# musyoku/chainer-speech-recognition

Measured on AMD Instinct MI355X. Metric: utterances/sec (T=1000, 40x3 feat, |V|~3000) CTC train step, higher is better.
Workload: dtype bf16

## Files before the change

chainer-speech-recognition_amd/asr/_lib.py:

```python
import ctypes
import os

import torch

_HERE = os.path.dirname(os.path.abspath(__file__))
_ACT = os.environ.get("ASR_ACT", "").lower()
LIB_PATH = os.environ.get("ASR_HIP_LIB") or os.path.join(os.path.dirname(_HERE),
                                                        "libasr_hip_f16.so" if _ACT in ("f16", "fp16", "float16", "half") else "libasr_hip.so")

_lib = None


def act_dtype():
    return torch.float16 if lib().asr_act_dtype() else torch.bfloat16


def debug_flag(key, default):
    for item in os.environ.get("ASR_DEBUG", "").split(","):
        k, _, v = item.strip().partition("=")
        if k == key and v:
            return int(v)
    return default

c_void_p, c_int, c_float, c_size_t = ctypes.c_void_p, ctypes.c_int, ctypes.c_float, ctypes.c_size_t
# ... 107 lines not shown
    "asr_gru_fwd_state": (c_int, [c_void_p] * 9 + [c_int] * 4 + [c_void_p]),
    "asr_gru_bwd_state": (c_int, [c_void_p] * 13 + [c_int] * 4 + [c_void_p, c_void_p]),
    "asr_sru_ws_bytes": (c_size_t, [c_int] * 3),
    "asr_sru_fwd": (c_int, [c_void_p] * 9 + [c_int] * 4 + [c_void_p, c_size_t]),
    "asr_sru_bwd": (c_int, [c_void_p] * 13 + [c_int] * 4 + [c_void_p, c_size_t]),
    "asr_sru_combine": (c_int, [c_void_p] * 5 + [c_longlong, c_int]),
    "asr_fill_f32": (c_int, [c_void_p, c_void_p, c_longlong, c_float]),
    "asr_sqnorm_acc": (c_int, [c_void_p, c_void_p, c_longlong, c_void_p]),
    "asr_clip_decay_sgd": (c_int, [c_void_p] * 4 + [c_longlong, c_int] + [c_float] * 5 + [c_void_p]),
    "asr_clip_decay_adam": (c_int, [c_void_p] * 5 + [c_longlong] + [c_float] * 7 + [c_void_p, c_int]),
    "asr_sqnorm_partials_count": (c_int, [c_longlong]),
    "asr_gather_abort": (c_int, [c_void_p, c_void_p, c_int, c_void_p, c_void_p]),
    "asr_step_control": (c_int, [c_void_p, c_void_p, c_longlong] + [c_void_p] * 3 + [c_float] * 5 + [c_void_p] * 2 + [c_int]),
    "asr_step_control_scaled": (c_int, [c_void_p, c_void_p, c_longlong] + [c_void_p] * 3 + [c_float] * 5 + [c_void_p] * 2 + [c_int, c_void_p]),
    "asr_adam_ctl": (c_int, [c_void_p] * 5 + [c_longlong] + [c_float] * 4 + [c_void_p]),
    "asr_crelu_fwd": (c_int, [c_void_p] * 3 + [c_longlong, c_int]),
    "asr_crelu_bwd": (c_int, [c_void_p] * 4 + [c_longlong, c_int]),
    "asr_softmax_fwd": (c_int, [c_void_p] * 3 + [c_longlong, c_int, c_int]),
    "asr_softmax_bwd": (c_int, [c_void_p] * 4 + [c_longlong, c_int, c_int]),
    "asr_avgpool_h_fwd": (c_int, [c_void_p] * 3 + [c_longlong, c_int, c_int, c_int]),
    "asr_avgpool_h_bwd": (c_int, [c_void_p] * 3 + [c_longlong, c_int, c_int, c_int]),
    "asr_unpool_h_fwd": (c_int, [c_void_p] * 3 + [c_longlong, c_int, c_int, c_int, c_int]),
    "asr_unpool_h_bwd": (c_int, [c_void_p] * 3 + [c_longlong, c_int, c_int, c_int, c_int]),
    "asr_gaussian_noise": (c_int, [c_void_p] * 3 + [c_longlong, c_float, ctypes.c_uint]),
    "asr_maxpool_h_indexes": (c_int, [c_void_p, c_void_p, c_void_p, c_longlong, c_int, c_int, c_int]),
    "asr_upsample_h_fwd": (c_int, [c_void_p] * 4 + [c_longlong] + [c_int] * 4),
    "asr_upsample_h_bwd": (c_int, [c_void_p] * 4 + [c_longlong] + [c_int] * 4),
    "asr_spp_bins": (c_int, [c_int]),
    "asr_spp_fwd": (c_int, [c_void_p] * 4 + [c_int] * 5),
    "asr_spp_bwd": (c_int, [c_void_p] * 4 + [c_int] * 5),
# ... 43 lines not shown
```

chainer-speech-recognition_amd/asr/_ops.py:

```python
import os

import torch

from . import _lib
from ._lib import check, ptr, stream

BF16 = _lib.act_dtype()
F32 = torch.float32


def _is_bf16(t):
    if t.dtype == BF16:
        return 1
    if t.dtype == F32:
        return 0
    raise TypeError("expected float32 or bfloat16, got %s" % t.dtype)


def gemm_nt(a, b, bias=None, out_dtype=BF16, out=None):
    assert a.dtype == BF16 and b.dtype == BF16 and a.dim() == 2 and b.dim() == 2
    assert a.stride(1) == 1 and b.stride(1) == 1 and a.shape[1] == b.shape[1]
    M, K = a.shape
    N = b.shape[0]
    if out is None:
# ... 503 lines not shown

def clip_decay_adam(p, g, m, v, alpha, beta1, beta2, eps, weight_decay, clip, grad_scale, sqnorm, step):
    rc = _lib.lib().asr_clip_decay_adam(stream(), ptr(p), ptr(g), ptr(m), ptr(v), p.numel(), alpha, beta1, beta2, eps,
                                        weight_decay, clip, grad_scale, ptr(sqnorm), int(step))
    check(rc, "asr_clip_decay_adam")


def abort_words():
    return [buf[1023:1024] for buf in _SYNC.values()]


_ABORT = {}


def gather_abort(dev, poison=None):
    words = [w for w in abort_words() if w.device == dev]
    ptrs = tuple(w.data_ptr() for w in words)
    st = _ABORT.get(dev.index)
    if st is None or st[0] != ptrs:
        table = torch.tensor(list(ptrs) or [0], dtype=torch.int64).to(dev)
        st = _ABORT[dev.index] = [ptrs, table, torch.zeros(1, dtype=torch.int32, device=dev) if st is None else st[2]]
    check(_lib.lib().asr_gather_abort(stream(), ptr(st[1]), len(words), ptr(st[2]), ptr(poison)), "asr_gather_abort")
    return st[2]


def clear_abort_words(dev):
    for w in abort_words():
        if w.device == dev:
            w.zero_()


def step_control(g, partials, clip, grad_scale, alpha, beta1, beta2, applied, ctl, any_abort=None, reserved_index=-1, loss_scale=None):
    if any_abort is None:
        any_abort = gather_abort(g.device)
    rc = _lib.lib().asr_step_control_scaled(stream(), ptr(g), g.numel(), ptr(partials), ptr(any_abort), None, float(clip),
                                            float(grad_scale), float(alpha), float(beta1), float(beta2), ptr(applied), ptr(ctl),
                                            int(reserved_index), None if loss_scale is None else ptr(loss_scale))
    check(rc, "asr_step_control_scaled")


def sqnorm_partials_count(n):
    return int(_lib.lib().asr_sqnorm_partials_count(int(n)))


def adam_ctl(p, g, m, v, beta1, beta2, eps, weight_decay, ctl):
    rc = _lib.lib().asr_adam_ctl(stream(), ptr(p), ptr(g), ptr(m), ptr(v), p.numel(), beta1, beta2, eps, weight_decay, ptr(ctl))
    check(rc, "asr_adam_ctl")


def sgd_ctl(p, g, v, kind, lr, momentum, weight_decay, ctl):
    rc = _lib.lib().asr_sgd_ctl(stream(), ptr(p), ptr(g), ptr(v), p.numel(), int(kind), lr, momentum, weight_decay, ptr(ctl))
    check(rc, "asr_sgd_ctl")


SRU_CHUNKED = [True]


def _sru_ws(T, B, D, dev):
    n = int(_lib.lib().asr_sru_ws_bytes(T, B, D)) if SRU_CHUNKED[0] else 0
    return (torch.empty(n, dtype=torch.uint8, device=dev), n) if n else (None, 0)


# ... 408 lines not shown
```

chainer-speech-recognition_amd/asr/functions.py:

```python
import math
import os

import torch

from . import _ops
from ._lib import debug_flag as _lib_debug
from .link import grad_buffer, grads_queued

BF16, F32 = _ops.BF16, torch.float32


_SIDE = {"streams": {}, "origins": {}, "enabled": True, "dirty": set(), "keep": [], "keep_bytes": 0,
         "join_before_recurrence": _lib_debug("side_join", 0) != 0}
_KEEP_LIMIT = 512
_KEEP_BYTES_LIMIT = int(_lib_debug("side_keep_gb", 48)) << 30


def side_stream():
    if not _SIDE["enabled"]:
        return None
    cur = torch.cuda.current_stream()
    key = cur.cuda_stream
    st = _SIDE["streams"].get(key)
    if st is None:
# ... 359 lines not shown


def conv_weight_matrix_bwd(W):
    return _ops.conv_weight_pack_bwd(W.contiguous())


def conv_weight_matrix_pad8(W):
    Co, Ci, KH, KW = W.shape
    Wp = torch.zeros((Co, 8, KH, KW), dtype=W.dtype, device=W.device)
    Wp[:, :Ci] = W
    return _ops.conv_weight_pack(Wp, Kp=(KH * KW * 8 + 31) // 32 * 32)


def convolution_2d(x, W, b, link, pad=(0, 0), causal=False, out_f32=False):
    pad_h, pad_t = (pad, pad) if isinstance(pad, int) else pad
    w16 = link.compute_copy("w16", W, conv_weight_matrix)
    w16t = link.compute_copy("w16t", W, conv_weight_matrix_t)
    wbwd = link.compute_copy("wbwd", W, conv_weight_matrix_bwd) if _ops.conv_implicit_ok(W.shape[0], W.shape[2], W.shape[3]) else None
    if x.dtype not in (F32, BF16):
        raise TypeError("convolution input must be float32 or bfloat16")
    w16p = link.compute_copy("w16p", W, conv_weight_matrix_pad8) if W.shape[1] < 8 else None
    y = _Conv2D.apply(x, W, b, w16, w16t, wbwd, w16p, int(pad_h), int(pad_t), bool(causal), bool(out_f32))
    return logical4(y)


def convolution_2d_given_weight(x, W, b, link, pad=(0, 0), causal=False, out_f32=False):
    pad_h, pad_t = (pad, pad) if isinstance(pad, int) else pad
    with torch.no_grad():
        w16 = conv_weight_matrix(W.detach())
        w16t = conv_weight_matrix_t(W.detach())
        wbwd = conv_weight_matrix_bwd(W.detach()) if _ops.conv_implicit_ok(W.shape[0], W.shape[2], W.shape[3]) else None
        w16p = conv_weight_matrix_pad8(W.detach()) if W.shape[1] < 8 else None
    y = _Conv2D.apply(x, W, b, w16, w16t, wbwd, w16p, int(pad_h), int(pad_t), bool(causal), bool(out_f32))
    return logical4(y)


# ... 51 lines not shown
        return False
    Co, Ci, KH, KW = wshape
    if not _ops.conv_mp_ok(Ci, KH, KW, Co, k) or Ci >= 8:
        return False
    return x.shape[2] + 2 * pad_h - KH + 1 >= 1 and (x.shape[3] if causal else x.shape[3] + 2 * pad_t - KW + 1) >= 1


def convolution_maxout_pool(x, W, b, link, pad, causal, k, given_weight=False):
    pad_h, pad_t = (pad, pad) if isinstance(pad, int) else pad
    if not convolution_maxout_pool_ok(x, tuple(W.shape), pad, causal, k):
        return None
    if given_weight:
        with torch.no_grad():
            w16q = conv_weight_matrix_pad8_128(W.detach())
    else:
        w16q = link.compute_copy("w16q", W, conv_weight_matrix_pad8_128)
    return logical4(_ConvMaxoutPool.apply(x, W, b, w16q, int(pad_h), int(pad_t), bool(causal), int(k)))


class _Dense(torch.autograd.Function):

    @staticmethod
    def forward(ctx, x2, W, b, w16, w16t, out_f32):
        y = _ops.gemm_nt(x2, w16, b.detach() if b is not None else None, F32 if out_f32 else BF16)
        ctx.save_for_backward(x2, w16t)
        ctx.params = (W, b)
        ctx.need_dx = ctx.needs_input_grad[0]
        if out_f32:
            ctx._asr_mailbox = _GradMailbox(y, b)
        return y

# ... 686 lines not shown
```

chainer-speech-recognition_amd/asr/link.py:

```python
import contextlib
import math

import torch

from . import _lib

F32 = torch.float32
BF16 = _lib.act_dtype()

_WEIGHT_EPOCH = [0]


def bump_weight_epoch():
    _WEIGHT_EPOCH[0] += 1


class Parameter(torch.nn.Parameter):

    def __new__(cls, data=None):
        if data is None:
            data = torch.empty(0, dtype=F32)
        return super().__new__(cls, data, requires_grad=True)


class Link(torch.nn.Module):
    def __init__(self):
        super().__init__()
        object.__setattr__(self, "_compute_cache", {})
        object.__setattr__(self, "_cast_registry", {})

    @contextlib.contextmanager
    def init_scope(self):
        yield

    @property
    def xp(self):
        return torch

    def params(self):
        return self.parameters()

    def namedparams(self):
        for name, p in self.named_parameters():
            yield "/" + name.replace(".", "/"), p
# ... 17 lines not shown
            src = state_dict.get(prefix + name)
            if p is not None and p.numel() == 0 and src is not None and src.numel() > 0:
                p.data = torch.empty(src.shape, dtype=p.dtype, device=p.device)
        super()._load_from_state_dict(state_dict, prefix, *args, **kwargs)
        bump_weight_epoch()

    def compute_copy(self, key, param, maker, layout=None):
        stamp = (_WEIGHT_EPOCH[0], param._version, param.data_ptr())
        hit = self._compute_cache.get(key)
        if hit is not None and hit[0] == stamp:
            _await_copy(hit)
            return hit[1]
        with torch.no_grad():
            value = maker(param.detach())
        self._compute_cache[key] = _made_copy(stamp, value)
        if layout is not None and value.is_cuda:
            self._cast_registry[key] = (param, value, _cast_jobs(param, layout))
        return value


def _made_copy(stamp, value):
    if not value.is_cuda:
        return (stamp, value, None, None)
    cur = torch.cuda.current_stream()
    return (stamp, value, {"stream": cur, "event": None}, {cur.cuda_stream})


def _await_copy(entry):
    if entry[2] is None:
        return
    cur = torch.cuda.current_stream()
# ... 9 lines not shown

def _cast_jobs(param, layout):
    n, shape = param.numel(), tuple(param.shape)
    if layout == "plain":
        return ((0, 0, n // shape[-1], shape[-1], 0),)
    if layout == "t_first":
        return ((0, 0, shape[0], n // shape[0], 1),)
    if layout == "t_last":
        return ((0, 0, n // shape[-1], shape[-1], 1),)
    if layout == "t_each":
        each = shape[-2] * shape[-1]
        return tuple((i * each, i * each, shape[-2], shape[-1], 1) for i in range(n // each))
    raise ValueError(layout)


def refresh_compute_copies(model):
    from . import _lib
    todo, sig = [], []
    for m in model.modules():
        reg = getattr(m, "_cast_registry", None)
        if not reg:
            continue
        for key, (param, out, jobs) in reg.items():
            hit = m._compute_cache.get(key)
            if hit is None or hit[1] is not out or hit[0][2] != param.data_ptr() or not param.is_cuda:
                continue
            todo.append((m, key, param, out))
            sig.append((param.data_ptr(), out.data_ptr(), jobs))
    if not todo:
        return 0
    cached = getattr(model, "_cast_table", None)
    if cached is None or cached[0] != sig:
        rows, tile = [], 0
        for src, dst, jobs in sig:
            for so, do, r, c, t in jobs:
                rows.append([src + 4 * so, dst + 2 * do, r, c, t, tile])
                tile += ((r + 63) // 64) * ((c + 63) // 64)
        table = torch.tensor(rows, dtype=torch.int64).to(todo[0][2].device)
        cached = (sig, table, len(rows), tile)
        object.__setattr__(model, "_cast_table", cached)
    _lib.check(_lib.lib().asr_cast_bf16_many(_lib.stream(), _lib.ptr(cached[1]), cached[2], cached[3]), "asr_cast_bf16_many")
    for m, key, param, out in todo:
        m._compute_cache[key] = _made_copy((_WEIGHT_EPOCH[0], param._version, param.data_ptr()), out)
    return cached[2]


class Chain(Link):
    pass


_GRAD_LISTENER = [None]


def grads_queued(*params):
    if _GRAD_LISTENER[0] is not None:
        _GRAD_LISTENER[0]([p for p in params if p is not None])


def grad_buffer(param):
# ... 89 lines not shown
```

chainer-speech-recognition_amd/asr/optimizers.py:

```python
import torch

from . import _ops
from .link import bump_weight_epoch, refresh_compute_copies

F32 = torch.float32
RESERVED = 64


class GradientClipping(object):
    name = "GradientClipping"

    def __init__(self, threshold):
        self.threshold = threshold


class WeightDecay(object):
    name = "WeightDecay"

    def __init__(self, rate):
        self.rate = rate


class Optimizer(object):
    def __init__(self):
# ... 51 lines not shown
                ls = self._loss_scale_buffer(loss.device)
                if ls is None:
                    loss.backward()
                else:
                    loss.backward(gradient=ls[0].reshape(loss.shape).to(loss.dtype))
            except BaseException:
                if self.communicator is not None:
                    self.communicator.abort_backward()
                from .functions import release_side_keeps
                release_side_keeps(to_allocator=True)
                raise
        self._ensure_flat()
        from .functions import join_side_stream
        join_side_stream()
        P, G = self._flat["P"], self._flat["G"]
        any_abort = _ops.gather_abort(G.device, G[0:1] if self.communicator is not None else None)
        scale = 1.0
        if self.communicator is not None:
            self.communicator.finish_backward(self)
            scale = 1.0 / self.communicator.size
        self.t += 1
        clip, decay = 0.0, 0.0
        for h in self._hooks:
            if isinstance(h, GradientClipping):
                clip = float(h.threshold)
            elif isinstance(h, WeightDecay):
                decay = float(h.rate)
        alpha, beta1, beta2 = self._control_constants()
        _ops.step_control(G, self._flat["partials"], clip, scale, alpha, beta1, beta2, self._flat["applied"], self._flat["ctl"],
                          any_abort, 0, self._loss_scale_buffer(G.device))
        self._step(P, G, decay, self._flat["ctl"])
        bump_weight_epoch()
        refresh_compute_copies(self.target)
        try:
            self._raise_if_previous_step_gave_up()
        finally:
            self._watch_gave_up()

    def _watch_gave_up(self):
        st = self._gave_up
        if st[0] is None:
            st[0] = torch.zeros(1, dtype=F32).pin_memory()
        if st[1] is None or st[1].query():
            st[0].copy_(self._flat["ctl"][6:7], non_blocking=True)
            st[1] = torch.cuda.Event()
            st[1].record()
            st[2] = self.t

# ... 91 lines not shown

    def _carried(self, total, dev, old, previous):
        state = torch.empty(total, dtype=F32, device=dev)
        _ops.fill_(state, 0.0)
        if old is not None and previous is not None and previous.device == dev:
            where = {pid: (o, n) for pid, o, n in zip(old["ids"], old["offsets"], old["numels"])}
            for pid, o, n in zip(self._flat["ids"], self._flat["offsets"], self._flat["numels"]):
                src = where.get(pid)
                if src is not None and src[1] == n:
                    state[o:o + n].copy_(previous[src[0]:src[0] + n])
        return state

    def _step(self, P, G, decay, ctl):
        raise NotImplementedError


class Adam(Optimizer):
    def __init__(self, alpha=0.001, beta1=0.9, beta2=0.999, eps=1e-8):
        super().__init__()
        self.alpha, self.beta1, self.beta2, self.eps = alpha, beta1, beta2, eps

        self.m = self.v = None

    def _init_state(self, total, dev, old):
        self.m = self._carried(total, dev, old, self.m)
        self.v = self._carried(total, dev, old, self.v)

    def _control_constants(self):
        return self.alpha, self.beta1, self.beta2

    def _state_buffers(self):
        return [self.m, self.v]

    def _step(self, P, G, decay, ctl):
        _ops.adam_ctl(P, G, self.m, self.v, self.beta1, self.beta2, self.eps, decay, ctl)


class SGD(Optimizer):
    kind = 0

    def __init__(self, lr=0.01):
        super().__init__()
        self.lr = lr
        self.momentum = 0.0
        self.vel = None

    def _init_state(self, total, dev, old):
        if self.kind:
            self.vel = self._carried(total, dev, old, self.vel)

    def _state_buffers(self):
        return [self.vel]

    def _step(self, P, G, decay, ctl):
        _ops.sgd_ctl(P, G, self.vel, self.kind, self.lr, self.momentum, decay, ctl)


class MomentumSGD(SGD):
    kind = 1

    def __init__(self, lr=0.01, momentum=0.9):
        super().__init__(lr)
        self.momentum = momentum


class NesterovAG(SGD):
    kind = 2

    def __init__(self, lr=0.01, momentum=0.9):
        super().__init__(lr)
# ... 55 lines not shown
```

chainer-speech-recognition_amd/csrc/optim.hip:

```cpp
#include "common.hpp"
#include "../../include/asr_hip.h"

namespace asr {
namespace optim {

__global__ __launch_bounds__(256) void sqnorm_kernel(const float* __restrict__ g, long long n, float* __restrict__ out) {
    __shared__ float scratch[32];
    float s = 0.f;
    for (long long i = blockIdx.x * (long long)blockDim.x + threadIdx.x; i < n; i += (long long)gridDim.x * blockDim.x) {
        const float v = g[i];
        s += v * v;
    }
    s = block_sum(s, scratch);
    if (threadIdx.x == 0) atomicAdd(out, s);
}

__global__ __launch_bounds__(256) void adam_kernel(float* __restrict__ p, const float* __restrict__ g,
                                                   float* __restrict__ m, float* __restrict__ v, long long n, float lr_t,
                                                   float beta1, float beta2, float eps, float decay, float clip,
                                                   float grad_scale, const float* __restrict__ sqnorm) {
    float rate = grad_scale;
    if (sqnorm) {
        if (!isfinite(sqnorm[0])) return;
        if (clip > 0.f) {
// ... 50 lines not shown
    if (threadIdx.x == 0) partials[blockIdx.x] = s;
}

__global__ void gather_abort_kernel(const long long* __restrict__ word_ptrs, int n, int* __restrict__ any_word, float* __restrict__ poison) {
    int any = 0;
    for (int i = 0; i < n; ++i) {
        const int* w = reinterpret_cast<const int*>(word_ptrs[i]);
        if (w && w[0] != 0) any = 1;
    }
    if (any_word) any_word[0] = any;
    if (any && poison) poison[0] = __int_as_float(0x7fc00000);
}

__global__ __launch_bounds__(256) void step_control_kernel(const float* __restrict__ partials, int npartials,
                                                           const int* __restrict__ abort0, const int* __restrict__ abort1,
                                                           float clip, float grad_scale, float alpha, float beta1, float beta2,
                                                           int* __restrict__ applied, float* __restrict__ ctl,
                                                           const float* __restrict__ reserved, float* __restrict__ ls) {
    __shared__ float scratch[32];
    float s = 0.f;
    for (int i = threadIdx.x; i < npartials; i += blockDim.x) s += partials[i];
    const float sq = block_sum(s, scratch);
    if (threadIdx.x != 0) return;
    ctl[4] = sq;
    const float* sqnorm = &sq;
    bool drop = !isfinite(sqnorm[0]);
    bool gave_up = false;
    if (abort0 && abort0[0] != 0) gave_up = true;
    if (abort1 && abort1[0] != 0) gave_up = true;
    if (reserved && !isfinite(reserved[0])) gave_up = true;
    if (gave_up) drop = true;
    if (ls) {
        grad_scale /= ls[0];
        if (drop && !gave_up) {
            if (ls[2] > 0.f) ls[0] = fmaxf(ls[0] * 0.5f, 1.f / 16777216.f);
            ls[1] = 0.f;
            ls[3] += 1.f;
        } else if (!drop) {
            ls[1] += 1.f;
            if (ls[2] > 0.f && ls[1] >= ls[2]) {
                ls[0] = fminf(ls[0] * 2.f, 16777216.f);
                ls[1] = 0.f;
// ... 6 lines not shown
        const float r = clip / norm;
        if (r < 1.f) rate *= r;
    }
    int t = applied[0];
    if (!drop) applied[0] = ++t;
    const double tt = t < 1 ? 1.0 : (double)t;
    const double fix1 = 1.0 - pow((double)beta1, tt), fix2 = 1.0 - pow((double)beta2, tt);
    ctl[0] = drop ? 1.f : 0.f;
    ctl[1] = rate;
    ctl[2] = (float)((double)alpha * sqrt(fix2) / fix1);
    ctl[3] = (float)t;
    ctl[5] = gave_up ? 1.f : 0.f;
    if (gave_up) ctl[6] += 1.f;
}

__global__ __launch_bounds__(256) void adam_ctl_kernel(float* __restrict__ p, const float* __restrict__ g, float* __restrict__ m,
                                                       float* __restrict__ v, long long n, float beta1, float beta2, float eps,
                                                       float decay, const float* __restrict__ ctl) {
    if (ctl[0] != 0.f) return;
    const float rate = ctl[1], lr_t = ctl[2];
    for (long long i = blockIdx.x * (long long)blockDim.x + threadIdx.x; i < n; i += (long long)gridDim.x * blockDim.x) {
        const float pi = p[i];
        const float gi = g[i] * rate + decay * pi;
        float mi = m[i], vi = v[i];
        mi += (1.f - beta1) * (gi - mi);
        vi += (1.f - beta2) * (gi * gi - vi);
        m[i] = mi;
        v[i] = vi;
        p[i] = pi - lr_t * mi / (sqrtf(vi) + eps);
    }
}

__global__ __launch_bounds__(256) void sgd_ctl_kernel(float* __restrict__ p, const float* __restrict__ g, float* __restrict__ v,
                                                      long long n, int kind, float lr, float mu, float decay,
                                                      const float* __restrict__ ctl) {
    if (ctl[0] != 0.f) return;
    const float rate = ctl[1];
    for (long long i = blockIdx.x * (long long)blockDim.x + threadIdx.x; i < n; i += (long long)gridDim.x * blockDim.x) {
        const float pi = p[i];
        const float gi = g[i] * rate + decay * pi;
        if (kind == 0) {
            p[i] = pi - lr * gi;
        } else {
            const float vi = mu * v[i] - lr * gi;
            v[i] = vi;
            p[i] = kind == 1 ? pi + vi : pi + mu * mu * vi - (1.f + mu) * lr * gi;
        }
    }
}

__global__ void fill_kernel(float* __restrict__ p, long long n, float value) {
    for (long long i = blockIdx.x * (long long)blockDim.x + threadIdx.x; i < n; i += (long long)gridDim.x * blockDim.x) p[i] = value;
}

}
}

using namespace asr;
using namespace asr::optim;

static inline int grid_for(long long n) {
// ... 35 lines not shown
    hipLaunchKernelGGL(sgd_kernel, dim3(grid_for(n)), dim3(256), 0, (hipStream_t)stream, p, g, v, n, kind, lr, momentum,
                       weight_decay, clip_threshold, grad_scale, sqnorm);
    ASR_LAUNCH_CHECK();
    return ASR_OK;
}

extern "C" int asr_sqnorm_partials_count(long long n) { return grid_for(n); }

extern "C" int asr_gather_abort(void* stream, const long long* word_ptrs, int n, int* any_word, float* poison) {
    if (n < 0 || (n > 0 && !word_ptrs) || (!any_word && !poison)) return ASR_ERR_BAD_ARG;
    hipLaunchKernelGGL(gather_abort_kernel, dim3(1), dim3(1), 0, (hipStream_t)stream, word_ptrs, n, any_word, poison);
    ASR_LAUNCH_CHECK();
    return ASR_OK;
}

extern "C" int asr_step_control_scaled(void* stream, const float* g, long long n, float* partials, const int* abort0, const int* abort1,
                                       float clip_threshold, float grad_scale, float alpha, float beta1, float beta2,
                                       int* applied_steps, float* ctl, int reserved_index, float* loss_scale) {
    if (!g || n <= 0 || !partials || !applied_steps || !ctl || reserved_index >= n) return ASR_ERR_BAD_ARG;
    const int blocks = grid_for(n);
    hipLaunchKernelGGL(sqnorm_partials_kernel, dim3(blocks), dim3(256), 0, (hipStream_t)stream, g, n, partials);
    hipLaunchKernelGGL(step_control_kernel, dim3(1), dim3(256), 0, (hipStream_t)stream, (const float*)partials, blocks, abort0,
                       abort1, clip_threshold, grad_scale, alpha, beta1, beta2, applied_steps, ctl,
                       reserved_index >= 0 ? g + reserved_index : (const float*)nullptr, loss_scale);
    ASR_LAUNCH_CHECK();
    return ASR_OK;
}

extern "C" int asr_step_control(void* stream, const float* g, long long n, float* partials, const int* abort0, const int* abort1,
                                float clip_threshold, float grad_scale, float alpha, float beta1, float beta2,
                                int* applied_steps, float* ctl, int reserved_index) {
    return asr_step_control_scaled(stream, g, n, partials, abort0, abort1, clip_threshold, grad_scale, alpha, beta1, beta2,
                                   applied_steps, ctl, reserved_index, nullptr);
}

extern "C" int asr_adam_ctl(void* stream, float* p, const float* g, float* m, float* v, long long n, float beta1, float beta2,
                            float eps, float weight_decay, const float* ctl) {
    if (!p || !g || !m || !v || !ctl || n <= 0) return ASR_ERR_BAD_ARG;
    hipLaunchKernelGGL(adam_ctl_kernel, dim3(grid_for(n)), dim3(256), 0, (hipStream_t)stream, p, g, m, v, n, beta1, beta2, eps,
                       weight_decay, ctl);
    ASR_LAUNCH_CHECK();
    return ASR_OK;
}

extern "C" int asr_sgd_ctl(void* stream, float* p, const float* g, float* v, long long n, int kind, float lr, float momentum,
                           float weight_decay, const float* ctl) {
    if (!p || !g || !ctl || n <= 0 || kind < 0 || kind > 2 || (kind > 0 && !v)) return ASR_ERR_BAD_ARG;
    hipLaunchKernelGGL(sgd_ctl_kernel, dim3(grid_for(n)), dim3(256), 0, (hipStream_t)stream, p, g, v, n, kind, lr, momentum,
                       weight_decay, ctl);
    ASR_LAUNCH_CHECK();
    return ASR_OK;
}
```

include/asr_hip.h:

```cpp
#ifndef ASR_HIP_H
#define ASR_HIP_H
#include <stddef.h>
#include <stdint.h>
#ifdef __cplusplus
extern "C" {
#endif

int asr_version(void);
int asr_act_dtype(void);
int asr_stream_delay(void* stream, int microseconds);
int asr_occupy_cus(void* stream, int microseconds, int lds_bytes, int blocks);
int asr_stream_traffic(void* stream, int microseconds, int lds_bytes, int blocks, void* buf, long long bytes);

size_t asr_ctc_workspace_bytes(int T, int B, int V, int Lmax, int gram);
int asr_ctc_forward(void* stream, const float* xs, const int32_t* label_unigram, const int32_t* label_bigram,
                    const int32_t* x_len, const int32_t* l_len, int T, int B, int V, int Lmax, int blank,
                    float* loss_per_utt, float* loss_mean, void* workspace, size_t workspace_bytes);
int asr_ctc_forward_lse(void* stream, const float* xs, const int32_t* label_unigram, const int32_t* label_bigram,
                        const int32_t* x_len, const int32_t* l_len, int T, int B, int V, int Lmax, int blank, float* loss_per_utt,
                        float* loss_mean, void* workspace, size_t workspace_bytes, const float* row_lse);
int asr_ctc_backward(void* stream, const float* xs, const int32_t* x_len, int T, int B, int V, int Lmax, int gram,
                     const float* gy, int gy_per_utt, float scale, float* grad, const void* workspace,
                     size_t workspace_bytes);
int asr_ctc_loss_grad(void* stream, const float* xs, const int32_t* label_unigram, const int32_t* label_bigram,
// ... 178 lines not shown
                        float grad_scale, const float* sqnorm, int step);
int asr_clip_decay_sgd(void* stream, float* p, const float* g, float* v, long long n, int kind, float lr, float momentum,
                       float weight_decay, float clip_threshold, float grad_scale, const float* sqnorm);
int asr_sqnorm_partials_count(long long n);
int asr_gather_abort(void* stream, const long long* word_ptrs, int n, int* any_word, float* poison);
int asr_step_control(void* stream, const float* g, long long n, float* partials, const int* abort0, const int* abort1,
                     float clip_threshold, float grad_scale, float alpha, float beta1, float beta2, int* applied_steps,
                     float* ctl, int reserved_index);
int asr_step_control_scaled(void* stream, const float* g, long long n, float* partials, const int* abort0, const int* abort1,
                            float clip_threshold, float grad_scale, float alpha, float beta1, float beta2, int* applied_steps,
                            float* ctl, int reserved_index, float* loss_scale);
int asr_adam_ctl(void* stream, float* p, const float* g, float* m, float* v, long long n, float beta1, float beta2, float eps,
                 float weight_decay, const float* ctl);
int asr_sgd_ctl(void* stream, float* p, const float* g, float* v, long long n, int kind, float lr, float momentum,
                float weight_decay, const float* ctl);

int asr_crelu_fwd(void* stream, const void* x, void* y, long long rows, int C);
int asr_crelu_bwd(void* stream, const void* x, const void* dy, void* dx, long long rows, int C);
int asr_softmax_fwd(void* stream, const void* x, void* y, long long rows, int C, int log_form);
int asr_softmax_bwd(void* stream, const void* y, const void* dy, void* dx, long long rows, int C, int log_form);
int asr_avgpool_h_fwd(void* stream, const void* x, void* y, long long R, int Hin, int C, int k);
int asr_avgpool_h_bwd(void* stream, const void* dy, void* dx, long long R, int Hin, int C, int k);
int asr_unpool_h_fwd(void* stream, const void* x, void* y, long long R, int Hin, int Hout, int C, int k);
int asr_unpool_h_bwd(void* stream, const void* dy, void* dx, long long R, int Hin, int Hout, int C, int k);
int asr_gaussian_noise(void* stream, const void* x, void* y, long long n, float stdv, unsigned int seed);
int asr_maxpool_h_indexes(void* stream, const void* x, void* idx_u8, long long R, int Hin, int C, int k);
int asr_upsample_h_fwd(void* stream, const void* x, const void* idx_u8, void* y, long long R, int Hin, int Hout, int C, int k);
int asr_upsample_h_bwd(void* stream, const void* dy, const void* idx_u8, void* dx, long long R, int Hin, int Hout, int C, int k);
int asr_spp_bins(int pyramid_height);
int asr_spp_fwd(void* stream, const void* x, void* y, int* pos, int T, int B, int H, int C, int pyramid_height);
// ... 7 lines not shown
```

Before: 2472.

## Fuse optimizer update with bf16 weight copy refresh and abort gather

Result: no change. 2486 (median of 6 runs) (+0.6%).

```diff
diff --git a/chainer-speech-recognition_amd/asr/_lib.py b/chainer-speech-recognition_amd/asr/_lib.py
--- a/chainer-speech-recognition_amd/asr/_lib.py
+++ b/chainer-speech-recognition_amd/asr/_lib.py
@@ -145,6 +145,9 @@
     "asr_step_control": (c_int, [c_void_p, c_void_p, c_longlong] + [c_void_p] * 3 + [c_float] * 5 + [c_void_p] * 2 + [c_int]),
     "asr_step_control_scaled": (c_int, [c_void_p, c_void_p, c_longlong] + [c_void_p] * 3 + [c_float] * 5 + [c_void_p] * 2 + [c_int, c_void_p]),
     "asr_adam_ctl": (c_int, [c_void_p] * 5 + [c_longlong] + [c_float] * 4 + [c_void_p]),
+    "asr_step_control_gather": (c_int, [c_void_p, c_void_p, c_longlong, c_void_p, c_void_p, c_int, c_void_p] + [c_float] * 5 + [c_void_p] * 2 + [c_int, c_void_p]),
+    "asr_adam_ctl_copies": (c_int, [c_void_p] * 5 + [c_float] * 4 + [c_void_p, c_void_p, c_int, c_longlong, c_void_p, c_int, c_longlong, c_void_p]),
+    "asr_sgd_ctl_copies": (c_int, [c_void_p] * 4 + [c_int] + [c_float] * 3 + [c_void_p, c_void_p, c_int, c_longlong, c_void_p, c_int, c_longlong, c_void_p]),
     "asr_crelu_fwd": (c_int, [c_void_p] * 3 + [c_longlong, c_int]),
     "asr_crelu_bwd": (c_int, [c_void_p] * 4 + [c_longlong, c_int]),
     "asr_softmax_fwd": (c_int, [c_void_p] * 3 + [c_longlong, c_int, c_int]),
diff --git a/chainer-speech-recognition_amd/asr/_ops.py b/chainer-speech-recognition_amd/asr/_ops.py
--- a/chainer-speech-recognition_amd/asr/_ops.py
+++ b/chainer-speech-recognition_amd/asr/_ops.py
@@ -541,14 +541,27 @@
 
 
 def gather_abort(dev, poison=None):
+    st, n = _abort_table(dev)
+    check(_lib.lib().asr_gather_abort(stream(), ptr(st[1]), n, ptr(st[2]), ptr(poison)), "asr_gather_abort")
+    return st[2]
+
+
+def _abort_table(dev):
     words = [w for w in abort_words() if w.device == dev]
     ptrs = tuple(w.data_ptr() for w in words)
     st = _ABORT.get(dev.index)
     if st is None or st[0] != ptrs:
         table = torch.tensor(list(ptrs) or [0], dtype=torch.int64).to(dev)
         st = _ABORT[dev.index] = [ptrs, table, torch.zeros(1, dtype=torch.int32, device=dev) if st is None else st[2]]
-    check(_lib.lib().asr_gather_abort(stream(), ptr(st[1]), len(words), ptr(st[2]), ptr(poison)), "asr_gather_abort")
-    return st[2]
+    return st, len(words)
+
+
+def step_control_gather(g, partials, clip, grad_scale, alpha, beta1, beta2, applied, ctl, reserved_index=-1, loss_scale=None):
+    st, n = _abort_table(g.device)
+    rc = _lib.lib().asr_step_control_gather(stream(), ptr(g), g.numel(), ptr(partials), ptr(st[1]), n, ptr(st[2]), float(clip),
+                                            float(grad_scale), float(alpha), float(beta1), float(beta2), ptr(applied), ptr(ctl),
+                                            int(reserved_index), None if loss_scale is None else ptr(loss_scale))
+    check(rc, "asr_step_control_gather")
 
 
 def clear_abort_words(dev):
@@ -573,6 +586,20 @@
 def adam_ctl(p, g, m, v, beta1, beta2, eps, weight_decay, ctl):
     rc = _lib.lib().asr_adam_ctl(stream(), ptr(p), ptr(g), ptr(m), ptr(v), p.numel(), beta1, beta2, eps, weight_decay, ptr(ctl))
     check(rc, "asr_adam_ctl")
+
+
+def _plan_args(plan):
+    return ptr(plan[1]) if plan[9] else None, plan[9], plan[3], ptr(plan[4]) if plan[5] else None, plan[5], plan[6], ptr(plan[7])
+
+
+def adam_ctl_copies(p, g, m, v, beta1, beta2, eps, weight_decay, ctl, plan):
+    rc = _lib.lib().asr_adam_ctl_copies(stream(), ptr(p), ptr(g), ptr(m), ptr(v), beta1, beta2, eps, weight_decay, ptr(ctl), *_plan_args(plan))
+    check(rc, "asr_adam_ctl_copies")
+
+
+def sgd_ctl_copies(p, g, v, kind, lr, momentum, weight_decay, ctl, plan):
+    rc = _lib.lib().asr_sgd_ctl_copies(stream(), ptr(p), ptr(g), ptr(v), int(kind), lr, momentum, weight_decay, ptr(ctl), *_plan_args(plan))
+    check(rc, "asr_sgd_ctl_copies")
 
 
 def sgd_ctl(p, g, v, kind, lr, momentum, weight_decay, ctl):
diff --git a/chainer-speech-recognition_amd/asr/functions.py b/chainer-speech-recognition_amd/asr/functions.py
--- a/chainer-speech-recognition_amd/asr/functions.py
+++ b/chainer-speech-recognition_amd/asr/functions.py
@@ -397,12 +397,15 @@
 
 def convolution_2d(x, W, b, link, pad=(0, 0), causal=False, out_f32=False):
     pad_h, pad_t = (pad, pad) if isinstance(pad, int) else pad
-    w16 = link.compute_copy("w16", W, conv_weight_matrix)
-    w16t = link.compute_copy("w16t", W, conv_weight_matrix_t)
-    wbwd = link.compute_copy("wbwd", W, conv_weight_matrix_bwd) if _ops.conv_implicit_ok(W.shape[0], W.shape[2], W.shape[3]) else None
+    K = W.shape[1] * W.shape[2] * W.shape[3]
+    w16 = link.compute_copy("w16", W, conv_weight_matrix, ("pack", 0, (K + 7) // 8 * 8, W.shape[1]))
+    w16t = link.compute_copy("w16t", W, conv_weight_matrix_t, ("pack", 1, (K + 7) // 8 * 8, W.shape[1]))
+    wbwd = link.compute_copy("wbwd", W, conv_weight_matrix_bwd, ("pack", 2, 0, W.shape[1])) \
+        if _ops.conv_implicit_ok(W.shape[0], W.shape[2], W.shape[3]) else None
     if x.dtype not in (F32, BF16):
         raise TypeError("convolution input must be float32 or bfloat16")
-    w16p = link.compute_copy("w16p", W, conv_weight_matrix_pad8) if W.shape[1] < 8 else None
+    w16p = link.compute_copy("w16p", W, conv_weight_matrix_pad8, ("pack", 0, (W.shape[2] * W.shape[3] * 8 + 31) // 32 * 32, 8)) \
+        if W.shape[1] < 8 else None
     y = _Conv2D.apply(x, W, b, w16, w16t, wbwd, w16p, int(pad_h), int(pad_t), bool(causal), bool(out_f32))
     return logical4(y)
 
@@ -484,7 +487,7 @@
         with torch.no_grad():
             w16q = conv_weight_matrix_pad8_128(W.detach())
     else:
-        w16q = link.compute_copy("w16q", W, conv_weight_matrix_pad8_128)
+        w16q = link.compute_copy("w16q", W, conv_weight_matrix_pad8_128, ("pack", 0, 128, 8))
     return logical4(_ConvMaxoutPool.apply(x, W, b, w16q, int(pad_h), int(pad_t), bool(causal), int(k)))
 
 
diff --git a/chainer-speech-recognition_amd/asr/link.py b/chainer-speech-recognition_amd/asr/link.py
--- a/chainer-speech-recognition_amd/asr/link.py
+++ b/chainer-speech-recognition_amd/asr/link.py
@@ -28,6 +28,7 @@
         super().__init__()
         object.__setattr__(self, "_compute_cache", {})
         object.__setattr__(self, "_cast_registry", {})
+        object.__setattr__(self, "_pack_registry", {})
 
     @contextlib.contextmanager
     def init_scope(self):
@@ -75,7 +76,9 @@
         with torch.no_grad():
             value = maker(param.detach())
         self._compute_cache[key] = _made_copy(stamp, value)
-        if layout is not None and value.is_cuda:
+        if isinstance(layout, tuple) and value.is_cuda:
+            self._pack_registry[key] = (param, value, tuple(int(v) for v in layout[1:]))
+        elif layout is not None and value.is_cuda:
             self._cast_registry[key] = (param, value, _cast_jobs(param, layout))
         return value
 
@@ -115,7 +118,7 @@
     raise ValueError(layout)
 
 
-def refresh_compute_copies(model):
+def refresh_compute_copies(model, skip=()):
     from . import _lib
     todo, sig = [], []
     for m in model.modules():
@@ -124,13 +127,13 @@
             continue
         for key, (param, out, jobs) in reg.items():
             hit = m._compute_cache.get(key)
-            if hit is None or hit[1] is not out or hit[0][2] != param.data_ptr() or not param.is_cuda:
+            if hit is None or hit[1] is not out or hit[0][2] != param.data_ptr() or not param.is_cuda or (id(m), key) in skip:
                 continue
             todo.append((m, key, param, out))
             sig.append((param.data_ptr(), out.data_ptr(), jobs))
     if not todo:
         return 0
-    cached = getattr(model, "_cast_table", None)
+    cached = getattr(model, "_cast_rest" if skip else "_cast_table", None)
     if cached is None or cached[0] != sig:
         rows, tile = [], 0
         for src, dst, jobs in sig:
@@ -139,11 +142,109 @@
                 tile += ((r + 63) // 64) * ((c + 63) // 64)
         table = torch.tensor(rows, dtype=torch.int64).to(todo[0][2].device)
         cached = (sig, table, len(rows), tile)
-        object.__setattr__(model, "_cast_table", cached)
+        object.__setattr__(model, "_cast_rest" if skip else "_cast_table", cached)
     _lib.check(_lib.lib().asr_cast_bf16_many(_lib.stream(), _lib.ptr(cached[1]), cached[2], cached[3]), "asr_cast_bf16_many")
     for m, key, param, out in todo:
         m._compute_cache[key] = _made_copy((_WEIGHT_EPOCH[0], param._version, param.data_ptr()), out)
     return cached[2]
+
+
+def copy_plan(total, mats, packs):
+    spans = [(o, r * c, None) for o, r, c, _, _ in mats]
+    spans += [(o, sh[0] * sh[1] * sh[2] * sh[3], i) for i, (o, sh, _) in enumerate(packs)]
+    jobs, tile = [], 0
+    for o, r, c, plain, trans in sorted(mats):
+        jobs.append([o, r, c, tile, plain, trans])
+        tile += ((r + 63) // 64) * ((c + 63) // 64)
+    ranges, block, cur = [], 0, 0
+
+    def span(offset, length, pack):
+        nonlocal block
+        if length > 0:
+            ranges.append([offset, length, block, pack])
+            block += (length + 1023) // 1024
+
+    for o, n, pack in sorted(spans, key=lambda x: x[0]):
+        if o < cur or n <= 0 or o + n > total:
+            raise ValueError("overlapping or empty spans in a copy plan")
+        span(cur, o - cur, -1)
+        if pack is not None:
+            span(o, n, pack)
+        cur = o + n
+    span(cur, total - cur, -1)
+    rows = []
+    for _, sh, dsts in packs:
+        if not 1 <= len(dsts) <= 4:
+            raise ValueError("a packed weight has one to four copies")
+        row = list(sh) + [len(dsts), 0, 0, 0]
+        for d in dsts:
+            row += list(d)
+        rows.append(row + [0] * (24 - len(row)))
+    return dict(jobs=jobs, tiles=tile, ranges=ranges, blocks=block, packs=rows)
+
+
+def _current(m, key, param, out):
+    hit = m._compute_cache.get(key)
+    return hit is not None and hit[1] is out and hit[0][2] == param.data_ptr() and param.is_cuda
+
+
+def update_plan(model, P):
+    base, total = P.data_ptr(), P.numel()
+    per_param, sig = {}, []
+    for m in model.modules():
+        for kind, reg in (("cast", getattr(m, "_cast_registry", None)), ("pack", getattr(m, "_pack_registry", None))):
+            for key, (param, out, what) in (reg or {}).items():
+                off = (param.data_ptr() - base) // 4
+                if not _current(m, key, param, out) or not param.is_contiguous() or off < 0 or off + param.numel() > total \
+                        or (param.data_ptr() - base) % 4 or param.device != P.device:
+                    continue
+                per_param.setdefault(id(param), (param, off, []))[2].append((kind, m, key, out, what))
+                sig.append((param.data_ptr(), out.data_ptr(), kind, what))
+    if not per_param:
+        return None
+    cached = getattr(model, "_cast_table", None)
+    if cached is not None and cached[0] == (base, total, sig):
+        return cached
+    mats, packs, entries = [], [], []
+    for param, off, copies in per_param.values():
+        casts = [c for c in copies if c[0] == "cast"]
+        pk = [c for c in copies if c[0] == "pack"][:4]
+        if casts and pk:
+            continue
+        if pk:
+            packs.append((off, tuple(param.shape), [(c[3].data_ptr(),) + tuple(c[4]) for c in pk]))
+            entries += [(c[1], c[2], param, c[3]) for c in pk]
+            continue
+        plain = next((c for c in casts if not c[4][0][4]), None)
+        trans = next((c for c in casts if c[4][0][4]), None)
+        split = (trans or plain)[4]
+        if sum(r * c for _, _, r, c, _ in split) != param.numel() or any(so != do for so, do, _, _, _ in split):
+            continue
+        for so, _, r, c, _ in split:
+            mats.append((off + so, r, c, plain[3].data_ptr() + 2 * so if plain else 0, trans[3].data_ptr() + 2 * so if trans else 0))
+        entries += [(c[1], c[2], param, c[3]) for c in (plain, trans) if c is not None]
+    plan = copy_plan(total, mats, packs)
+
+    def table(rows, width):
+        return torch.tensor(rows or [[0] * width], dtype=torch.int64).to(P.device)
+
+    cached = ((base, total, sig), table(plan["jobs"], 6), len(entries), plan["tiles"], table(plan["ranges"], 4), len(plan["ranges"]),
+              plan["blocks"], table(plan["packs"], 24), entries, len(plan["jobs"]))
+    object.__setattr__(model, "_cast_table", cached)
+    return cached
+
+
+def copies_written(model, plan, was_current):
+    covered = set()
+    for (m, key, param, out), ok in zip(plan[8], was_current):
+        covered.add((id(m), key))
+        if ok:
+            m._compute_cache[key] = _made_copy((_WEIGHT_EPOCH[0], param._version, param.data_ptr()), out)
+    refresh_compute_copies(model, covered)
+
+
+def copies_current(plan):
+    return [m._compute_cache[key][0] == (_WEIGHT_EPOCH[0], param._version, param.data_ptr()) for m, key, param, out in plan[8]]
 
 
 class Chain(Link):
diff --git a/chainer-speech-recognition_amd/asr/optimizers.py b/chainer-speech-recognition_amd/asr/optimizers.py
--- a/chainer-speech-recognition_amd/asr/optimizers.py
+++ b/chainer-speech-recognition_amd/asr/optimizers.py
@@ -1,7 +1,7 @@
 import torch
 
 from . import _ops
-from .link import bump_weight_epoch, refresh_compute_copies
+from .link import bump_weight_epoch, copies_current, copies_written, refresh_compute_copies, update_plan
 
 F32 = torch.float32
 RESERVED = 64
@@ -89,9 +89,9 @@
         from .functions import join_side_stream
         join_side_stream()
         P, G = self._flat["P"], self._flat["G"]
-        any_abort = _ops.gather_abort(G.device, G[0:1] if self.communicator is not None else None)
         scale = 1.0
         if self.communicator is not None:
+            any_abort = _ops.gather_abort(G.device, G[0:1])
             self.communicator.finish_backward(self)
             scale = 1.0 / self.communicator.size
         self.t += 1
@@ -102,11 +102,22 @@
             elif isinstance(h, WeightDecay):
                 decay = float(h.rate)
         alpha, beta1, beta2 = self._control_constants()
-        _ops.step_control(G, self._flat["partials"], clip, scale, alpha, beta1, beta2, self._flat["applied"], self._flat["ctl"],
-                          any_abort, 0, self._loss_scale_buffer(G.device))
-        self._step(P, G, decay, self._flat["ctl"])
-        bump_weight_epoch()
-        refresh_compute_copies(self.target)
+        if self.communicator is not None:
+            _ops.step_control(G, self._flat["partials"], clip, scale, alpha, beta1, beta2, self._flat["applied"], self._flat["ctl"],
+                              any_abort, 0, self._loss_scale_buffer(G.device))
+        else:
+            _ops.step_control_gather(G, self._flat["partials"], clip, scale, alpha, beta1, beta2, self._flat["applied"],
+                                     self._flat["ctl"], 0, self._loss_scale_buffer(G.device))
+        plan = update_plan(self.target, P)
+        if plan is None:
+            self._step(P, G, decay, self._flat["ctl"])
+            bump_weight_epoch()
+            refresh_compute_copies(self.target)
+        else:
+            current = copies_current(plan)
+            self._step_copies(P, G, decay, self._flat["ctl"], plan)
+            bump_weight_epoch()
+            copies_written(self.target, plan, current)
         try:
             self._raise_if_previous_step_gave_up()
         finally:
@@ -228,6 +239,9 @@
     def _step(self, P, G, decay, ctl):
         raise NotImplementedError
 
+    def _step_copies(self, P, G, decay, ctl, plan):
+        raise NotImplementedError
+
 
 class Adam(Optimizer):
     def __init__(self, alpha=0.001, beta1=0.9, beta2=0.999, eps=1e-8):
@@ -248,6 +262,9 @@
 
     def _step(self, P, G, decay, ctl):
         _ops.adam_ctl(P, G, self.m, self.v, self.beta1, self.beta2, self.eps, decay, ctl)
+
+    def _step_copies(self, P, G, decay, ctl, plan):
+        _ops.adam_ctl_copies(P, G, self.m, self.v, self.beta1, self.beta2, self.eps, decay, ctl, plan)
 
 
 class SGD(Optimizer):
@@ -268,6 +285,9 @@
 
     def _step(self, P, G, decay, ctl):
         _ops.sgd_ctl(P, G, self.vel, self.kind, self.lr, self.momentum, decay, ctl)
+
+    def _step_copies(self, P, G, decay, ctl, plan):
+        _ops.sgd_ctl_copies(P, G, self.vel, self.kind, self.lr, self.momentum, decay, ctl, plan)
 
 
 class MomentumSGD(SGD):
diff --git a/chainer-speech-recognition_amd/csrc/optim.hip b/chainer-speech-recognition_amd/csrc/optim.hip
--- a/chainer-speech-recognition_amd/csrc/optim.hip
+++ b/chainer-speech-recognition_amd/csrc/optim.hip
@@ -88,6 +88,7 @@
 
 __global__ __launch_bounds__(256) void step_control_kernel(const float* __restrict__ partials, int npartials,
                                                            const int* __restrict__ abort0, const int* __restrict__ abort1,
+                                                           const long long* __restrict__ word_ptrs, int nwords, int* __restrict__ any_word,
                                                            float clip, float grad_scale, float alpha, float beta1, float beta2,
                                                            int* __restrict__ applied, float* __restrict__ ctl,
                                                            const float* __restrict__ reserved, float* __restrict__ ls) {
@@ -100,6 +101,15 @@
     const float* sqnorm = &sq;
     bool drop = !isfinite(sqnorm[0]);
     bool gave_up = false;
+    if (word_ptrs) {
+        int any = 0;
+        for (int i = 0; i < nwords; ++i) {
+            const int* w = reinterpret_cast<const int*>(word_ptrs[i]);
+            if (w && w[0] != 0) any = 1;
+        }
+        if (any_word) any_word[0] = any;
+        if (any) gave_up = true;
+    }
     if (abort0 && abort0[0] != 0) gave_up = true;
     if (abort1 && abort1[0] != 0) gave_up = true;
     if (reserved && !isfinite(reserved[0])) gave_up = true;
@@ -136,20 +146,36 @@
     if (gave_up) ctl[6] += 1.f;
 }
 
+__device__ __forceinline__ float pin(float x) {
+    asm("" : "+v"(x));
+    return x;
+}
+__device__ __forceinline__ float adam_element(float pi, float g, float& mi, float& vi, float rate, float lr_t, float beta1, float beta2,
+                                              float eps, float decay) {
+    const float gi = pin(g * rate) + pin(decay * pi);
+    mi = mi + pin((1.f - beta1) * (gi - mi));
+    vi = __builtin_fmaf(1.f - beta2, __builtin_fmaf(gi, gi, -vi), vi);
+    return pi - pin(lr_t * mi) / (sqrtf(vi) + eps);
+}
+__device__ __forceinline__ float sgd_element(float pi, float g, float& v0, int kind, float rate, float lr, float mu, float decay) {
+    const float gi = __builtin_fmaf(decay, pi, pin(g * rate));
+    if (kind == 0) return __builtin_fmaf(-lr, gi, pi);
+    const float vi = __builtin_fmaf(mu, v0, -pin(lr * gi));
+    v0 = vi;
+    return kind == 1 ? pi + vi : (pi + pin(pin(mu * mu) * vi)) - pin(pin((1.f + mu) * lr) * gi);
+}
+
 __global__ __launch_bounds__(256) void adam_ctl_kernel(float* __restrict__ p, const float* __restrict__ g, float* __restrict__ m,
                                                        float* __restrict__ v, long long n, float beta1, float beta2, float eps,
                                                        float decay, const float* __restrict__ ctl) {
     if (ctl[0] != 0.f) return;
     const float rate = ctl[1], lr_t = ctl[2];
     for (long long i = blockIdx.x * (long long)blockDim.x + threadIdx.x; i < n; i += (long long)gridDim.x * blockDim.x) {
-        const float pi = p[i];
-        const float gi = g[i] * rate + decay * pi;
         float mi = m[i], vi = v[i];
-        mi += (1.f - beta1) * (gi - mi);
-        vi += (1.f - beta2) * (gi * gi - vi);
+        const float x = adam_element(p[i], g[i], mi, vi, rate, lr_t, beta1, beta2, eps, decay);
         m[i] = mi;
         v[i] = vi;
-        p[i] = pi - lr_t * mi / (sqrtf(vi) + eps);
+        p[i] = x;
     }
 }
 
@@ -159,14 +185,194 @@
     if (ctl[0] != 0.f) return;
     const float rate = ctl[1];
     for (long long i = blockIdx.x * (long long)blockDim.x + threadIdx.x; i < n; i += (long long)gridDim.x * blockDim.x) {
-        const float pi = p[i];
-        const float gi = g[i] * rate + decay * pi;
-        if (kind == 0) {
-            p[i] = pi - lr * gi;
+        float vi = kind ? v[i] : 0.f;
+        const float x = sgd_element(p[i], g[i], vi, kind, rate, lr, mu, decay);
+        if (kind) v[i] = vi;
+        p[i] = x;
+    }
+}
+
+struct AdamRule {
+    float* __restrict__ m;
+    float* __restrict__ v;
+    float beta1, beta2, eps, decay, rate, lr_t;
+    __device__ __forceinline__ void control(const float* __restrict__ ctl) { rate = ctl[1]; lr_t = ctl[2]; }
+    __device__ __forceinline__ float load0(long long i) const { return m[i]; }
+    __device__ __forceinline__ float load1(long long i) const { return v[i]; }
+    __device__ __forceinline__ float4 load0v(long long i) const { return *(const float4*)(m + i); }
+    __device__ __forceinline__ float4 load1v(long long i) const { return *(const float4*)(v + i); }
+    __device__ __forceinline__ void store0(long long i, float x) const { m[i] = x; }
+    __device__ __forceinline__ void store1(long long i, float x) const { v[i] = x; }
+    __device__ __forceinline__ void store0v(long long i, float4 x) const { *(float4*)(m + i) = x; }
+    __device__ __forceinline__ void store1v(long long i, float4 x) const { *(float4*)(v + i) = x; }
+    __device__ __forceinline__ float apply(float pi, float g, float& mi, float& vi) const {
+        return adam_element(pi, g, mi, vi, rate, lr_t, beta1, beta2, eps, decay);
+    }
+};
+
+struct SgdRule {
+    float* __restrict__ v;
+    int kind;
+    float lr, mu, decay, rate;
+    __device__ __forceinline__ void control(const float* __restrict__ ctl) { rate = ctl[1]; }
+    __device__ __forceinline__ float load0(long long i) const { return kind ? v[i] : 0.f; }
+    __device__ __forceinline__ float load1(long long) const { return 0.f; }
+    __device__ __forceinline__ float4 load0v(long long i) const { return kind ? *(const float4*)(v + i) : make_float4(0.f, 0.f, 0.f, 0.f); }
+    __device__ __forceinline__ float4 load1v(long long) const { return make_float4(0.f, 0.f, 0.f, 0.f); }
+    __device__ __forceinline__ void store0(long long i, float x) const { if (kind) v[i] = x; }
+    __device__ __forceinline__ void store1(long long, float) const {}
+    __device__ __forceinline__ void store0v(long long i, float4 x) const { if (kind) *(float4*)(v + i) = x; }
+    __device__ __forceinline__ void store1v(long long, float4) const {}
+    __device__ __forceinline__ float apply(float pi, float g, float& v0, float&) const {
+        return sgd_element(pi, g, v0, kind, rate, lr, mu, decay);
+    }
+};
+
+__device__ __forceinline__ int plan_find(const long long* __restrict__ table, int n, int stride, int at, long long x, long long* keys) {
+    if (n <= 256) {
+        if ((int)threadIdx.x < n) keys[threadIdx.x] = table[threadIdx.x * stride + at];
+        __syncthreads();
+        int lo = 0, hi = n - 1;
+        while (lo < hi) {
+            const int mid = (lo + hi + 1) >> 1;
+            if (keys[mid] <= x) lo = mid; else hi = mid - 1;
+        }
+        return lo;
+    }
+    int lo = 0, hi = n - 1;
+    while (lo < hi) {
+        const int mid = (lo + hi + 1) >> 1;
+        if (table[mid * stride + at] <= x) lo = mid; else hi = mid - 1;
+    }
+    return lo;
+}
+
+__device__ __forceinline__ void store_packed(const long long* __restrict__ pk, long long e, float x) {
+    const long long Co = pk[0];
+    const int Ci = (int)pk[1], KH = (int)pk[2], KW = (int)pk[3], nd = (int)pk[4];
+    long long r = e;
+    const int kw = (int)(r % KW); r /= KW;
+    const int kh = (int)(r % KH); r /= KH;
+    const int ci = (int)(r % Ci);
+    const int co = (int)(r / Ci);
+    const uint16_t h = f32_to_bf16(x);
+    for (int d = 0; d < nd; ++d) {
+        uint16_t* __restrict__ dst = (uint16_t*)pk[8 + 4 * d];
+        const int mode = (int)pk[9 + 4 * d];
+        const long long Kp = pk[10 + 4 * d], Cp = pk[11 + 4 * d];
+        const long long k = (long long)(kh * KW + kw) * Cp + ci;
+        if (mode == 0) { if (k < Kp) dst[(long long)co * Kp + k] = h; }
+        else if (mode == 1) { if (k < Kp) dst[k * Co + co] = h; }
+        else dst[((long long)(ci * KH + kh) * KW + kw) * Co + co] = h;
+    }
+}
+
+template <typename Rule>
+__global__ __launch_bounds__(256) void update_copies_kernel(float* __restrict__ p, const float* __restrict__ g, Rule rule,
+                                                            const float* __restrict__ ctl, const long long* __restrict__ jobs,
+                                                            int njobs, long long total_tiles, const long long* __restrict__ ranges,
+                                                            int nranges, const long long* __restrict__ packs) {
+    __shared__ float tile[64][65];
+    __shared__ long long keys[256];
+    if (ctl[0] != 0.f) return;
+    rule.control(ctl);
+    if ((long long)blockIdx.x >= total_tiles) {
+        const long long blk = (long long)blockIdx.x - total_tiles;
+        const int j = plan_find(ranges, nranges, 4, 2, blk, keys);
+        const long long off = ranges[j * 4 + 0], len = ranges[j * 4 + 1], pack = ranges[j * 4 + 3];
+        const long long e0 = (blk - ranges[j * 4 + 2]) * 1024;
+        for (int k = 0; k < 4; ++k) {
+            const long long e = e0 + k * 256 + threadIdx.x;
+            if (e >= len) break;
+            const long long i = off + e;
+            float s0 = rule.load0(i), s1 = rule.load1(i);
+            const float x = rule.apply(p[i], g[i], s0, s1);
+            rule.store0(i, s0);
+            rule.store1(i, s1);
+            p[i] = x;
+            if (pack >= 0) store_packed(packs + pack * 24, e, x);
+        }
+        return;
+    }
+    const int j = plan_find(jobs, njobs, 6, 3, (long long)blockIdx.x, keys);
+    const long long off = jobs[j * 6 + 0];
+    const int rows = (int)jobs[j * 6 + 1], cols = (int)jobs[j * 6 + 2];
+    const int local = (int)((long long)blockIdx.x - jobs[j * 6 + 3]);
+    uint16_t* __restrict__ plain = (uint16_t*)jobs[j * 6 + 4];
+    uint16_t* __restrict__ trans = (uint16_t*)jobs[j * 6 + 5];
+    const int tiles_c = (cols + 63) / 64;
+    const int r0 = (local / tiles_c) * 64, c0 = (local % tiles_c) * 64;
+    const int tx = threadIdx.x & 15, ty = threadIdx.x >> 4;
+    const int c = c0 + tx * 4;
+    float x[4][4];
+    if ((cols & 3) == 0) {
+        float4 pv[4], gv[4], s0[4], s1[4];
+#pragma unroll
+        for (int q = 0; q < 4; ++q) {
+            const int r = r0 + ty + 16 * q;
+            if (r < rows && c < cols) {
+                const long long i = off + (long long)r * cols + c;
+                pv[q] = *(const float4*)(p + i);
+                gv[q] = *(const float4*)(g + i);
+                s0[q] = rule.load0v(i);
+                s1[q] = rule.load1v(i);
+            }
+        }
+#pragma unroll
+        for (int q = 0; q < 4; ++q) {
+            const int r = r0 + ty + 16 * q;
+            x[q][0] = x[q][1] = x[q][2] = x[q][3] = 0.f;
+            if (r < rows && c < cols) {
+                const long long i = off + (long long)r * cols + c;
+                x[q][0] = rule.apply(pv[q].x, gv[q].x, s0[q].x, s1[q].x);
+                x[q][1] = rule.apply(pv[q].y, gv[q].y, s0[q].y, s1[q].y);
+                x[q][2] = rule.apply(pv[q].z, gv[q].z, s0[q].z, s1[q].z);
+                x[q][3] = rule.apply(pv[q].w, gv[q].w, s0[q].w, s1[q].w);
+                rule.store0v(i, s0[q]);
+                rule.store1v(i, s1[q]);
+                *(float4*)(p + i) = make_float4(x[q][0], x[q][1], x[q][2], x[q][3]);
+                if (plain) {
+                    uint2 o;
+                    o.x = (unsigned)f32_to_bf16(x[q][0]) | ((unsigned)f32_to_bf16(x[q][1]) << 16);
+                    o.y = (unsigned)f32_to_bf16(x[q][2]) | ((unsigned)f32_to_bf16(x[q][3]) << 16);
+                    *(uint2*)(plain + (size_t)r * cols + c) = o;
+                }
+            }
+        }
+    } else {
+#pragma unroll
+        for (int q = 0; q < 4; ++q) {
+            const int r = r0 + ty + 16 * q;
+            for (int k = 0; k < 4; ++k) {
+                x[q][k] = 0.f;
+                if (r < rows && c + k < cols) {
+                    const long long i = off + (long long)r * cols + c + k;
+                    float s0 = rule.load0(i), s1 = rule.load1(i);
+                    x[q][k] = rule.apply(p[i], g[i], s0, s1);
+                    rule.store0(i, s0);
+                    rule.store1(i, s1);
+                    p[i] = x[q][k];
+                    if (plain) plain[(size_t)r * cols + c + k] = f32_to_bf16(x[q][k]);
+                }
+            }
+        }
+    }
+    if (!trans) return;
+#pragma unroll
+    for (int q = 0; q < 4; ++q)
+        for (int k = 0; k < 4; ++k) tile[ty + 16 * q][tx * 4 + k] = x[q][k];
+    __syncthreads();
+    const bool vecr = (rows & 3) == 0;
+    for (int i = ty; i < 64; i += 16) {
+        const int cc = c0 + i, r = r0 + tx * 4;
+        if (cc >= cols || r >= rows) continue;
+        if (vecr) {
+            uint2 o;
+            o.x = (unsigned)f32_to_bf16(tile[tx * 4 + 0][i]) | ((unsigned)f32_to_bf16(tile[tx * 4 + 1][i]) << 16);
+            o.y = (unsigned)f32_to_bf16(tile[tx * 4 + 2][i]) | ((unsigned)f32_to_bf16(tile[tx * 4 + 3][i]) << 16);
+            *(uint2*)(trans + (size_t)cc * rows + r) = o;
         } else {
-            const float vi = mu * v[i] - lr * gi;
-            v[i] = vi;
-            p[i] = kind == 1 ? pi + vi : pi + mu * mu * vi - (1.f + mu) * lr * gi;
+            for (int k = 0; k < 4 && r + k < rows; ++k) trans[(size_t)cc * rows + r + k] = f32_to_bf16(tile[tx * 4 + k][i]);
         }
     }
 }
@@ -232,17 +438,32 @@
     return ASR_OK;
 }
 
-extern "C" int asr_step_control_scaled(void* stream, const float* g, long long n, float* partials, const int* abort0, const int* abort1,
-                                       float clip_threshold, float grad_scale, float alpha, float beta1, float beta2,
-                                       int* applied_steps, float* ctl, int reserved_index, float* loss_scale) {
+static int step_control(void* stream, const float* g, long long n, float* partials, const int* abort0, const int* abort1,
+                        const long long* word_ptrs, int nwords, int* any_word, float clip_threshold, float grad_scale, float alpha,
+                        float beta1, float beta2, int* applied_steps, float* ctl, int reserved_index, float* loss_scale) {
     if (!g || n <= 0 || !partials || !applied_steps || !ctl || reserved_index >= n) return ASR_ERR_BAD_ARG;
     const int blocks = grid_for(n);
     hipLaunchKernelGGL(sqnorm_partials_kernel, dim3(blocks), dim3(256), 0, (hipStream_t)stream, g, n, partials);
     hipLaunchKernelGGL(step_control_kernel, dim3(1), dim3(256), 0, (hipStream_t)stream, (const float*)partials, blocks, abort0,
-                       abort1, clip_threshold, grad_scale, alpha, beta1, beta2, applied_steps, ctl,
+                       abort1, word_ptrs, nwords, any_word, clip_threshold, grad_scale, alpha, beta1, beta2, applied_steps, ctl,
                        reserved_index >= 0 ? g + reserved_index : (const float*)nullptr, loss_scale);
     ASR_LAUNCH_CHECK();
     return ASR_OK;
+}
+
+extern "C" int asr_step_control_scaled(void* stream, const float* g, long long n, float* partials, const int* abort0, const int* abort1,
+                                       float clip_threshold, float grad_scale, float alpha, float beta1, float beta2,
+                                       int* applied_steps, float* ctl, int reserved_index, float* loss_scale) {
+    return step_control(stream, g, n, partials, abort0, abort1, nullptr, 0, nullptr, clip_threshold, grad_scale, alpha, beta1, beta2,
+                        applied_steps, ctl, reserved_index, loss_scale);
+}
+
+extern "C" int asr_step_control_gather(void* stream, const float* g, long long n, float* partials, const long long* word_ptrs, int nwords,
+                                       int* any_word, float clip_threshold, float grad_scale, float alpha, float beta1, float beta2,
+                                       int* applied_steps, float* ctl, int reserved_index, float* loss_scale) {
+    if (nwords < 0 || (nwords > 0 && !word_ptrs)) return ASR_ERR_BAD_ARG;
+    return step_control(stream, g, n, partials, nullptr, nullptr, word_ptrs, nwords, any_word, clip_threshold,
+                        grad_scale, alpha, beta1, beta2, applied_steps, ctl, reserved_index, loss_scale);
 }
 
 extern "C" int asr_step_control(void* stream, const float* g, long long n, float* partials, const int* abort0, const int* abort1,
@@ -269,3 +490,33 @@
     ASR_LAUNCH_CHECK();
     return ASR_OK;
 }
+
+static int plan_ok(const long long* jobs, int njobs, long long total_tiles, const long long* ranges, int nranges, long long total_blocks) {
+    if (njobs < 0 || nranges < 0 || total_tiles < 0 || total_blocks < 0 || (njobs > 0 && !jobs) || (nranges > 0 && !ranges)) return 0;
+    if ((njobs == 0) != (total_tiles == 0) || (nranges == 0) != (total_blocks == 0)) return 0;
+    const long long grid = total_tiles + total_blocks;
+    return grid > 0 && grid < (1ll << 31);
+}
+
+extern "C" int asr_adam_ctl_copies(void* stream, float* p, const float* g, float* m, float* v, float beta1, float beta2, float eps,
+                                   float weight_decay, const float* ctl, const long long* jobs, int njobs, long long total_tiles,
+                                   const long long* ranges, int nranges, long long total_blocks, const long long* packs) {
+    if (!p || !g || !m || !v || !ctl || !plan_ok(jobs, njobs, total_tiles, ranges, nranges, total_blocks)) return ASR_ERR_BAD_ARG;
+    AdamRule rule{m, v, beta1, beta2, eps, weight_decay, 0.f, 0.f};
+    hipLaunchKernelGGL(update_copies_kernel<AdamRule>, dim3((unsigned)(total_tiles + total_blocks)), dim3(256), 0, (hipStream_t)stream,
+                       p, g, rule, ctl, jobs, njobs, total_tiles, ranges, nranges, packs);
+    ASR_LAUNCH_CHECK();
+    return ASR_OK;
+}
+
+extern "C" int asr_sgd_ctl_copies(void* stream, float* p, const float* g, float* v, int kind, float lr, float momentum,
+                                  float weight_decay, const float* ctl, const long long* jobs, int njobs, long long total_tiles,
+                                  const long long* ranges, int nranges, long long total_blocks, const long long* packs) {
+    if (!p || !g || !ctl || kind < 0 || kind > 2 || (kind > 0 && !v) || !plan_ok(jobs, njobs, total_tiles, ranges, nranges, total_blocks))
+        return ASR_ERR_BAD_ARG;
+    SgdRule rule{v, kind, lr, momentum, weight_decay, 0.f};
+    hipLaunchKernelGGL(update_copies_kernel<SgdRule>, dim3((unsigned)(total_tiles + total_blocks)), dim3(256), 0, (hipStream_t)stream,
+                       p, g, rule, ctl, jobs, njobs, total_tiles, ranges, nranges, packs);
+    ASR_LAUNCH_CHECK();
+    return ASR_OK;
+}
diff --git a/include/asr_hip.h b/include/asr_hip.h
--- a/include/asr_hip.h
+++ b/include/asr_hip.h
@@ -216,6 +216,15 @@
                  float weight_decay, const float* ctl);
 int asr_sgd_ctl(void* stream, float* p, const float* g, float* v, long long n, int kind, float lr, float momentum,
                 float weight_decay, const float* ctl);
+int asr_step_control_gather(void* stream, const float* g, long long n, float* partials, const long long* word_ptrs, int nwords,
+                            int* any_word, float clip_threshold, float grad_scale, float alpha, float beta1, float beta2,
+                            int* applied_steps, float* ctl, int reserved_index, float* loss_scale);
+int asr_adam_ctl_copies(void* stream, float* p, const float* g, float* m, float* v, float beta1, float beta2, float eps,
+                        float weight_decay, const float* ctl, const long long* jobs, int njobs, long long total_tiles,
+                        const long long* ranges, int nranges, long long total_blocks, const long long* packs);
+int asr_sgd_ctl_copies(void* stream, float* p, const float* g, float* v, int kind, float lr, float momentum, float weight_decay,
+                       const float* ctl, const long long* jobs, int njobs, long long total_tiles, const long long* ranges,
+                       int nranges, long long total_blocks, const long long* packs);
 
 int asr_crelu_fwd(void* stream, const void* x, void* y, long long rows, int C);
 int asr_crelu_bwd(void* stream, const void* x, const void* dy, void* dx, long long rows, int C);
```
